# barlettacarmen/CrCNN

Hardware: AMD Instinct MI355X
Metric: encrypted images/sec (higher is better)
Workload: dtype u64

## Files before the change

crcnn_amd/csrc/abi.hip:

```cpp
#include <cstdlib>
#include <cstring>
#include "kernels.h"
#include "chacha.h"
#include "work_arena.h"

#define CHECK_CTX(c) do { if (!(c) || (c)->device < 0) return CRC_ERR_INVALID_ARGUMENT; \
        int dev_ = -1; if (hipGetDevice(&dev_) != hipSuccess || dev_ != (c)->device) HIPCHK(hipSetDevice((c)->device)); } while (0)
#define RUN(x) do { int rc_ = (x); if (rc_) return rc_; } while (0)
static inline hipStream_t S(void *s) { return (hipStream_t)s; }
static inline bool form_ok(int f) { return f == CRC_COEFF || f == CRC_NTT; }
static inline bool nform_ok(int f) { return f == CRC_COEFF || f == CRC_NTT || f == CRC_NTTP; }
static inline bool lform_ok(int f) { return nform_ok(f) || f == CRC_NTTL; }
static inline bool limb_in(int f) { return f == CRC_NTTL || f == CRC_NTTLS; }
static inline u64 *work_base(void *d_work) { return WorkArena(d_work).take<u64>(0); }
static inline size_t work_bytes(size_t words) { WorkArena a; a.take<u64>(words); return a.bytes(); }

extern "C" int crc_plain_to_ntt(crc_ctx *c, const uint64_t *d_plain, size_t count, uint64_t *d_out, void *stream)
{
    CHECK_CTX(c); if (!d_plain || !d_out) return CRC_ERR_INVALID_ARGUMENT;
    return k_plain_ntt(c, d_plain, count, 1, true, d_out, S(stream));
}
extern "C" int crc_plain_expand(crc_ctx *c, const uint64_t *d_compact, size_t count, uint64_t *d_plain, void *stream)
{
    CHECK_CTX(c); if (!d_compact || !d_plain) return CRC_ERR_INVALID_ARGUMENT;
// ... 324 lines not shown
    if (!d_w || !d_bias_ntt || !d_w_out || !d_bias_out || nf < 1 || zd < 1 || xf < 1 || yf < 1 || cxs < 1 || cys < 1 || pxf < 1 ||
        pyf < 1) return CRC_ERR_INVALID_ARGUMENT;
    return k_fold_pool(c, d_w, d_bias_ntt, d_div_ntt, d_w_out, d_bias_out, nf, zd, xf, yf, cxs, cys, pxf, pyf, S(stream));
}
extern "C" int crc_conv2d_hoist_pool(crc_ctx *c, const uint64_t *d_w, const uint64_t *d_bias_ntt, const uint64_t *d_div_ntt, int nf, int zd, int xf, int yf,
                                     int pxf, int pyf, uint64_t *d_w_out, uint64_t *d_bias_out, void *stream)
{
    CHECK_CTX(c);
    if (!d_w || !d_bias_ntt || !d_w_out || !d_bias_out || nf < 1 || zd < 1 || xf < 1 || yf < 1 || pxf < 1 || pyf < 1) return CRC_ERR_INVALID_ARGUMENT;
    return k_fold_pool(c, d_w, d_bias_ntt, d_div_ntt, d_w_out, d_bias_out, nf, zd, xf, yf, 1, 1, pxf, pyf, S(stream), true);
}

extern "C" int crc_pool(crc_ctx *c, const uint64_t *d_x, int B, int zd, int xd, int yd, int xs, int ys, int xf, int yf,
                        const uint64_t *d_div, int form, uint64_t *d_y, void *stream)
{
    CHECK_CTX(c);
    if (!d_x || !d_y || B < 0 || zd < 1 || !nform_ok(form) || !conv_shape_ok(xd, yd, xs, ys, xf, yf)) return CRC_ERR_INVALID_ARGUMENT;
    if (B == 0) return CRC_OK;
    hipStream_t st = S(stream);
    const int xo = (xd - xf) / xs + 1, yo = (yd - yf) / ys + 1;
    if (form == CRC_NTTP) return k_pool(c, d_x, d_y, B, zd, xd, yd, xs, ys, xf, yf, d_div, st, 1);
    if (form == CRC_NTT || !d_div) return k_pool(c, d_x, d_y, B, zd, xd, yd, xs, ys, xf, yf, form == CRC_NTT ? d_div : nullptr, st);
    RUN(k_pool(c, d_x, d_y, B, zd, xd, yd, xs, ys, xf, yf, nullptr, st));
    const size_t cnt = (size_t)B * zd * xo * yo;
    RUN(k_ntt_ct(c, false, d_y, d_y, cnt, 2, false, st, nullptr, 0, 0));
    RUN(k_rowwise(c, d_y, d_div, cnt, 2, 2, 1, cnt, 0, st));
    return k_ntt_ct(c, true, d_y, d_y, cnt, 2, false, st, nullptr, 0, 0);
}

extern "C" int crc_pad(crc_ctx *c, const uint64_t *d_x, int B, int zd, int xd, int yd, int px0, int px1, int py0, int py1, int form, uint64_t *d_y,
                       void *stream)
{
    CHECK_CTX(c);
    if (!d_x || !d_y || B < 0 || zd < 1 || xd < 1 || yd < 1 || px0 < 0 || px1 < 0 || py0 < 0 || py1 < 0 || !form_ok(form)) return CRC_ERR_INVALID_ARGUMENT;
    if (((uintptr_t)d_x | (uintptr_t)d_y) & 15) return CRC_ERR_INVALID_ARGUMENT;
    const long long xo = (long long)xd + px0 + px1, yo = (long long)yd + py0 + py1;
    if (xo > 0x7fffffffLL || yo > 0x7fffffffLL) return CRC_ERR_INVALID_ARGUMENT;
    const size_t ctb = crc_ct_words(c, 2) * 8;
    const size_t in_bytes = (size_t)B * zd * xd * yd * ctb, out_bytes = (size_t)B * zd * (size_t)xo * (size_t)yo * ctb;
    const uintptr_t x0 = (uintptr_t)d_x, y0 = (uintptr_t)d_y;
    if (x0 < y0 + out_bytes && y0 < x0 + in_bytes) return CRC_ERR_INVALID_ARGUMENT;
    if (B == 0) return CRC_OK;
    return k_pad(c, d_x, d_y, B, zd, xd, yd, px0, px1, py0, py1, S(stream));
}

extern "C" int crc_batchnorm(crc_ctx *c, uint64_t *d_x, int B, int zd, int xd, int yd, const uint64_t *d_mean, const uint64_t *d_invstd,
                             int form, void *stream)
{
    CHECK_CTX(c);
    if (!d_x || !d_mean || !d_invstd || B < 0 || zd < 1 || xd < 1 || yd < 1 || !form_ok(form)) return CRC_ERR_INVALID_ARGUMENT;
    if (B == 0) return CRC_OK;
    hipStream_t st = S(stream);
    const size_t hw = (size_t)xd * yd, cnt = (size_t)B * zd * hw;
    if (form == CRC_NTT) return k_bn_ntt(c, d_x, B, zd, (int)hw, d_mean, d_invstd, st);
    RUN(k_rowwise(c, d_x, d_mean, cnt, 2, 1, -1, hw, (size_t)zd, st));
    RUN(k_ntt_ct(c, false, d_x, d_x, cnt, 2, false, st, nullptr, 0, 0));
    RUN(k_rowwise(c, d_x, d_invstd, cnt, 2, 2, 1, hw, (size_t)zd, st));
    return k_ntt_ct(c, true, d_x, d_x, cnt, 2, false, st, nullptr, 0, 0);
}

extern "C" int crc_plan_mac(const crc_ctx *c, int zd, int xd, int yd, int xs, int ys, int xf, int yf, int nf, int B, int matrix_cores, int *w_form)
{
    if (!c || !w_form || zd < 1 || nf < 1 || !conv_shape_ok(xd, yd, xs, ys, xf, yf)) return CRC_ERR_INVALID_ARGUMENT;
    bool packable = true;
    for (int i = 0; i < c->k; i++) if (c->tabs[i].m.bits > 55) packable = false;
    *w_form = packable ? CRC_NTTP : CRC_NTT;
    if (!matrix_cores || !packable) return CRC_OK;
    if (zd == 1) { if (k_limb_conv1_shape(c, zd, xd, yd, xs, ys, xf, yf, nf)) *w_form = CRC_NTTL1; return CRC_OK; }
    const int min_steps = c->tune.mfma_min_steps > 0 ? c->tune.mfma_min_steps : 8;
    const long long P = (long long)((xd - xf) / xs + 1) * ((yd - yf) / ys + 1);
    const long long rows = (long long)B * 2 * P, min_rows = nf >= 24 ? 32 : 64;
    const bool few_filters_ok = nf >= 24 || (long long)c->n * c->k <= 32768;
    if (zd >= 16 && few_filters_ok && (long long)((zd + 31) / 32) * xf * yf >= min_steps && crc_limb_supported(c, zd, xf, yf) && (B <= 0 ||
        rows >= min_rows)) *w_form = CRC_NTTL;
    return CRC_OK;
}
extern "C" size_t crc_scalar_weights_bytes(const crc_ctx *c, int nf, int zd, int xf, int yf)
{
    return c && nf >= 1 && zd >= 1 && xf >= 1 && yf >= 1 ? k_scalar_weights_bytes(c, nf, zd, xf, yf) : 0;
}
extern "C" int crc_scalar_supported(const crc_ctx *c, int B, int zd, int xd, int yd, int xs, int ys, int xf, int yf, int nf)
{
    if (!c || B < 1 || zd < 1 || nf < 1 || !conv_shape_ok(xd, yd, xs, ys, xf, yf)) return 0;
    return k_scalar_supported(c, B, zd, xd, yd, xs, ys, xf, yf, nf) ? 1 : 0;
}
extern "C" int crc_scalar_pack_weights(crc_ctx *c, const uint64_t *d_w, int w_stride, int nf, int zd, int xf, int yf, void *d_ws, int *constant, void *stream)
{
    if (constant) *constant = 1;
    CHECK_CTX(c);
    if (!d_w || !d_ws || !constant || nf < 1 || zd < 1 || xf < 1 || yf < 1 || (w_stride != 1 && w_stride != c->n)) return CRC_ERR_INVALID_ARGUMENT;
    if (c->k > 8 || !k_limb_supported(c, k_limb_steps(zd, xf, yf) * 32)) return CRC_ERR_UNSUPPORTED;
    return k_scalar_pack_weights(c, d_w, (size_t)w_stride, (signed char *)d_ws, nf, zd, xf, yf, constant, S(stream));
}
extern "C" int crc_plan_mac_scalar(const crc_ctx *c, int zd, int xd, int yd, int xs, int ys, int xf, int yf, int nf, int B, int *w_form)
{
    RUN(crc_plan_mac(c, zd, xd, yd, xs, ys, xf, yf, nf, B, 1, w_form));
    if (c->tune.scalar_mac && zd >= 2 && k_scalar_supported(c, B < 1 ? 1 : B, zd, xd, yd, xs, ys, xf, yf, nf)) *w_form = CRC_NTTLS;
    return CRC_OK;
}
extern "C" int crc_plan_fold_pool(const crc_ctx *c, int zd, int xd, int yd, int xs, int ys, int xf, int yf, int nf, int pxs, int pys, int pxf, int pyf,
    int *fold)
{
    if (!c || !fold || zd < 1 || nf < 1 || !conv_shape_ok(xd, yd, xs, ys, xf, yf) || pxs < 1 || pys < 1 || pxf < 1 || pyf < 1) return CRC_ERR_INVALID_ARGUMENT;
    *fold = 0;
    const int xo = (xd - xf) / xs + 1, yo = (yd - yf) / ys + 1;
    const int xf2 = (pxf - 1) * xs + xf, yf2 = (pyf - 1) * ys + yf, xs2 = xs * pxs, ys2 = ys * pys;
    if (xf2 > xd || yf2 > yd || pxf > xo || pyf > yo) return CRC_OK;
    const int xo2 = (xd - xf2) / xs2 + 1, yo2 = (yd - yf2) / ys2 + 1;
    if (xo2 != (xo - pxf) / pxs + 1 || yo2 != (yo - pyf) / pys + 1) return CRC_OK;
    const long long fpad = (nf + 7) / 8 * 8, T1 = (long long)zd * xf * yf, T2 = (long long)zd * xf2 * yf2;
    const long long cost_sep = fpad * xo * yo * (T1 + 24) + (long long)nf * xo2 * yo2 * 10 * (pxf * pyf + 1);
    const long long cost_fused = fpad * xo2 * yo2 * (T2 + 24);
    *fold = cost_fused < cost_sep ? 1 : 0;
    return CRC_OK;
}

static long long plan_mac_cost(const crc_ctx *c, int zd, int xd, int yd, int xs, int ys, int xf, int yf, int nf, int B, int matrix_cores)
{
    int wf = CRC_NTT;
    if (crc_plan_mac(c, zd, xd, yd, xs, ys, xf, yf, nf, B, matrix_cores, &wf) != CRC_OK) return -1;
    const long long P = (long long)((xd - xf) / xs + 1) * ((yd - yf) / ys + 1);
    if (wf == CRC_NTTL1) return 32 * ((2 * P + 15) / 16 * 8) * ((k_limb_conv1_form(c, xf, yf, nf) == 2 ? 40 : 64) + 24) * 8 / 5;
    if (wf == CRC_NTTL) return (long long)(nf + 31) / 32 * 32 * P * ((long long)k_limb_steps(zd, xf, yf) * 32 + 24);
    return (long long)(nf + 7) / 8 * 8 * P * ((long long)zd * xf * yf + 24);
}
extern "C" int crc_plan_hoist_pool(const crc_ctx *c, int uzd, int uxd, int uyd, int uxs, int uys, int uxf, int uyf, int unf, int zd, int xd, int yd, int xs,
                                   int ys, int xf, int yf, int nf, int pxs, int pys, int pxf, int pyf, int B, int matrix_cores, int *hoist)
{
    if (!c || !hoist || zd < 1 || nf < 1 || !conv_shape_ok(xd, yd, xs, ys, xf, yf) || pxs < 1 || pys < 1 || pxf < 1 || pyf < 1) return CRC_ERR_INVALID_ARGUMENT;
    *hoist = 0;
    if (!c->tune.hoist_pool || xs != 1 || ys != 1 || pxs * pys == 1) return CRC_OK;
    int fold = 0;
    { const int rc = crc_plan_fold_pool(c, zd, xd, yd, xs, ys, xf, yf, nf, pxs, pys, pxf, pyf, &fold); if (rc != CRC_OK) return rc; }
    if (!fold) return CRC_OK;
    if (uzd < 1 || unf != zd || !conv_shape_ok(uxd, uyd, uxs, uys, uxf, uyf) || (uxd - uxf) / uxs + 1 != xd || (uyd - uyf) / uys + 1 != yd) return CRC_OK;
    const int uxf2 = (pxf - 1) * uxs + uxf, uyf2 = (pyf - 1) * uys + uyf, sxd = xd - pxf + 1, syd = yd - pyf + 1;
    if (uxf2 > uxd || uyf2 > uyd || !conv_shape_ok(uxd, uyd, uxs, uys, uxf2, uyf2)) return CRC_OK;
    if ((uxd - uxf2) / uxs + 1 != sxd || (uyd - uyf2) / uys + 1 != syd) return CRC_OK;
    const int xo = xd - xf + 1, yo = yd - yf + 1;
    if (!conv_shape_ok(sxd, syd, pxs, pys, xf, yf) || (sxd - xf) / pxs + 1 != (xo - pxf) / pxs + 1 || (syd - yf) / pys + 1 != (yo - pyf) / pys + 1) return CRC_OK;
    int uf = CRC_NTT, uf2 = CRC_NTT;
    if (crc_plan_mac(c, uzd, uxd, uyd, uxs, uys, uxf, uyf, unf, B, matrix_cores, &uf) != CRC_OK) return CRC_OK;
    if (crc_plan_mac(c, uzd, uxd, uyd, uxs, uys, uxf2, uyf2, unf, B, matrix_cores, &uf2) != CRC_OK) return CRC_OK;
    if ((uf == CRC_NTTL1 || uf == CRC_NTTL) && uf2 != uf) return CRC_OK;
    const int xf2 = xf + pxf - 1, yf2 = yf + pyf - 1;
    const long long folded = plan_mac_cost(c, uzd, uxd, uyd, uxs, uys, uxf, uyf, unf, B, matrix_cores) +
                             plan_mac_cost(c, zd, xd, yd, pxs, pys, xf2, yf2, nf, B, matrix_cores);
    const long long hoisted = plan_mac_cost(c, uzd, uxd, uyd, uxs, uys, uxf2, uyf2, unf, B, matrix_cores) +
                              plan_mac_cost(c, zd, sxd, syd, pxs, pys, xf, yf, nf, B, matrix_cores);
    *hoist = hoisted < folded ? 1 : 0;
    return CRC_OK;
}

#define PLAN_BOX_READ 21
extern "C" int crc_plan_conv1_box(const crc_ctx *c, int zd, int xd, int yd, int xs, int ys, int xf, int yf, int nf, int bxf, int byf, int B, int matrix_cores,
                                  int *box)
{
    if (!c || !box || zd < 1 || nf < 1 || bxf < 1 || byf < 1 || !conv_shape_ok(xd, yd, xs, ys, xf, yf)) return CRC_ERR_INVALID_ARGUMENT;
    *box = 0;
    if (!c->tune.conv1_box || !matrix_cores || bxf * byf == 1) return CRC_OK;
    if (!crc_limb_conv1_box_supported(c, zd, xd, yd, xs, ys, xf, yf, nf, bxf, byf)) return CRC_OK;
    const int xf2 = (bxf - 1) * xs + xf, yf2 = (byf - 1) * ys + yf, xdi = xd - (bxf - 1) * xs, ydi = yd - (byf - 1) * ys;
    if (!conv_shape_ok(xd, yd, xs, ys, xf2, yf2)) return CRC_OK;
    int wf = CRC_NTT;
    if (crc_plan_mac(c, zd, xdi, ydi, xs, ys, xf, yf, nf, B, matrix_cores, &wf) != CRC_OK || wf != CRC_NTTL1) return CRC_OK;
    const long long enlarged = plan_mac_cost(c, zd, xd, yd, xs, ys, xf2, yf2, nf, B, matrix_cores);
    const long long boxed = plan_mac_cost(c, zd, xdi, ydi, xs, ys, xf, yf, nf, B, matrix_cores) +
                            (long long)xdi * ydi * 2 * (bxf * byf - 1) * PLAN_BOX_READ;
    *box = enlarged >= 0 && boxed < enlarged ? 1 : 0;
    return CRC_OK;
}

static size_t square_chunk(const crc_ctx *c)
{
    if (c->tune.sq_chunk > 0) return (size_t)c->tune.sq_chunk;
    const size_t nk = (size_t)c->n * c->k;
    return nk <= 32768 ? 1024 : nk <= 65536 ? 512 : nk <= 131072 ? 256 : 128;
}

struct ActWork { u64 *xh, *s, *kp, *y3, *rest; size_t step; };
enum { ACT_XH = 1, ACT_S = 2, ACT_MULTIPLY = 4 };
static ActWork act_layout(const crc_ctx *c, size_t planes, size_t pin, size_t pout, int dbc, int regions, WorkArena &a)
{
    ActWork L{};
    L.step = square_chunk(c) / pin ? square_chunk(c) / pin : 1;
    const size_t pp = planes < L.step ? planes : L.step, cin = pp * pin, cout = pp * pout;
    const size_t pr = regions & ACT_MULTIPLY ? k_multiply_work_words(c, cin) : k_square_work_words(c, cin), rl = k_relin_work_words(c, cout, dbc);
    if (regions & ACT_XH) L.xh = a.take<u64>(cin * crc_ct_words(c, 2));
    if (regions & ACT_S) L.s = a.take<u64>(cin * crc_ct_words(c, 2));
    L.kp = a.take<u64>(k_relin_keys_words(c, dbc));
    L.y3 = a.take<u64>(cin * crc_ct_words(c, 3));
    L.rest = a.take<u64>(pr > rl ? pr : rl);
    return L;
}
static size_t act_bytes(const crc_ctx *c, size_t planes, size_t pin, size_t pout, int dbc, int regions)
{
    WorkArena a;
    act_layout(c, planes, pin, pout, dbc, regions, a);
    return a.bytes();
}
static inline size_t pass_len(size_t count, size_t o, size_t step) { return count - o < step ? count - o : step; }
static int ntt_copy(crc_ctx *c, const u64 *x, size_t ch, u64 *xh, void *stream)
{
    HIPCHK(hipMemcpyAsync(xh, x, 8 * ch * crc_ct_words(c, 2), hipMemcpyDeviceToDevice, S(stream)));
    return crc_ntt_fwd(c, xh, ch, 2, stream);
}
extern "C" size_t crc_square_relin_work_bytes(const crc_ctx *c, size_t count, int dbc) { return c && dbc_ok(dbc) ? act_bytes(c, count, 1, 1, dbc, 0) : 0; }
extern "C" size_t crc_encrypt_dev_work_bytes(const crc_ctx *c, size_t count) { return c ? work_bytes(k_encrypt_work_words(c, count)) : 0; }
extern "C" int crc_encrypt_dev_key(crc_ctx *c, const uint64_t *d_pk, const uint64_t *d_plain, size_t count, const uint8_t *key, uint64_t stream_base,
                                   uint64_t *d_ct, void *d_work, void *stream)
{
    return crc_encrypt_dev_key_forms(c, d_pk, d_plain, count, key, stream_base, CRC_COEFF, d_ct, d_work, stream);
}
extern "C" int crc_encrypt_dev(crc_ctx *c, const uint64_t *d_pk, const uint64_t *d_plain, size_t count, uint64_t seed, uint64_t *d_ct, void *d_work,
    void *stream)
{
    return crc_encrypt_dev_forms(c, d_pk, d_plain, count, seed, CRC_COEFF, d_ct, d_work, stream);
}
extern "C" int crc_encrypt_dev_key_forms(crc_ctx *c, const uint64_t *d_pk, const uint64_t *d_plain, size_t count, const uint8_t *key, uint64_t stream_base,
                                         int out_form, uint64_t *d_ct, void *d_work, void *stream)
{
    CHECK_CTX(c); if (!d_pk || !d_plain || !d_ct || !d_work || !key || (out_form != CRC_COEFF && out_form != CRC_NTT)) return CRC_ERR_INVALID_ARGUMENT;
    return k_encrypt(c, d_pk, d_plain, count, chacha_load_key(key), stream_base, d_ct, work_base(d_work), S(stream), out_form == CRC_NTT);
}
extern "C" int crc_encrypt_dev_forms(crc_ctx *c, const uint64_t *d_pk, const uint64_t *d_plain, size_t count, uint64_t seed, int out_form, uint64_t *d_ct,
                                     void *d_work, void *stream)
{
    CHECK_CTX(c); if (!d_pk || !d_plain || !d_ct || !d_work || (out_form != CRC_COEFF && out_form != CRC_NTT)) return CRC_ERR_INVALID_ARGUMENT;
    return k_encrypt(c, d_pk, d_plain, count, chacha_seed_key(seed), 0, d_ct, work_base(d_work), S(stream), out_form == CRC_NTT);
}
extern "C" void crc_encrypt_dev_noise_thresholds(uint64_t *h_out19) { if (h_out19) k_encrypt_cdt(h_out19); }

static bool ct_form_ok(int f) { return f == CRC_COEFF || f == CRC_NTT; }
extern "C" size_t crc_decrypt_dev_work_bytes(const crc_ctx *c, size_t count, int size, int in_form)
{
    return c && ct_form_ok(in_form) ? work_bytes(k_decrypt_work_words(c, count, size, in_form == CRC_NTT)) : 0;
}
extern "C" int crc_decrypt_dev(crc_ctx *c, const uint64_t *d_sk, const uint64_t *d_ct, size_t count, int size, int in_form, uint64_t *d_plain, void *d_work,
                               void *stream)
{
    CHECK_CTX(c); if (!d_sk || !d_ct || !d_plain || !d_work || !ct_form_ok(in_form)) return CRC_ERR_INVALID_ARGUMENT;
    return k_decrypt(c, d_sk, d_ct, count, size, in_form == CRC_NTT, d_plain, work_base(d_work), S(stream));
}
extern "C" size_t crc_noise_budget_dev_work_bytes(const crc_ctx *c, size_t count, int size, int in_form)
{
    return c && ct_form_ok(in_form) && (size == 2 || size == 3) ? work_bytes(k_decrypt_work_words(c, count, size, in_form == CRC_NTT)) : 0;
}
extern "C" int crc_noise_budget_dev(crc_ctx *c, const uint64_t *d_sk, const uint64_t *d_ct, size_t count, int size, int in_form, int32_t *d_bits, int32_t *d_min,
                                    void *d_work, void *stream)
{
    if (!d_sk || !d_ct || !d_bits || !d_work || !ct_form_ok(in_form) || size < 2 || size > 3) return CRC_ERR_INVALID_ARGUMENT;
    CHECK_CTX(c);
    return k_noise_budget(c, d_sk, d_ct, count, size, in_form == CRC_NTT, d_bits, d_min, work_base(d_work), S(stream));
}
extern "C" int crc_budget_bits_host(const crc_ctx *c, const uint64_t *h_v, size_t count, int32_t *h_bits)
{
    if (!c || !h_v || !h_bits) return CRC_ERR_INVALID_ARGUMENT;
    return k_budget_bits_host(c, h_v, count, h_bits);
}
static int slots_args_ok(const crc_ctx *c, const void *values, const void *plain, int slots, size_t item_stride, size_t slot_stride)
{
    if (!crc_slots_supported(c)) return CRC_ERR_PARAMETERS;
    if (!values || !plain || slots < 1 || slots > c->n || !item_stride || !slot_stride) return CRC_ERR_INVALID_ARGUMENT;
    return CRC_OK;
}
extern "C" int crc_slots_compose(crc_ctx *c, const int64_t *h_values, size_t count, int slots, size_t item_stride, size_t slot_stride, uint64_t *h_plain)
{
    if (!c) return CRC_ERR_INVALID_ARGUMENT;
    RUN(slots_args_ok(c, h_values, h_plain, slots, item_stride, slot_stride));
    return k_slots_compose_host(c, (const long long *)h_values, count, slots, item_stride, slot_stride, h_plain);
}
extern "C" int crc_slots_decompose(crc_ctx *c, const uint64_t *h_plain, size_t count, int slots, int64_t *h_values, size_t item_stride, size_t slot_stride)
{
    if (!c) return CRC_ERR_INVALID_ARGUMENT;
    RUN(slots_args_ok(c, h_values, h_plain, slots, item_stride, slot_stride));
    return k_slots_decompose_host(c, h_plain, count, slots, (long long *)h_values, item_stride, slot_stride);
}
extern "C" int crc_slots_compose_dev(crc_ctx *c, const int64_t *d_values, size_t count, int slots, size_t item_stride, size_t slot_stride, uint64_t *d_plain,
                                     void *stream)
{
    CHECK_CTX(c);
    RUN(slots_args_ok(c, d_values, d_plain, slots, item_stride, slot_stride));
    if (((uintptr_t)d_plain & 15) || ((uintptr_t)d_values & 7)) return CRC_ERR_INVALID_ARGUMENT;
    return k_slots_compose(c, (const long long *)d_values, count, slots, item_stride, slot_stride, d_plain, S(stream));
}
extern "C" int crc_slots_decompose_dev(crc_ctx *c, const uint64_t *d_plain, size_t count, int slots, int64_t *d_values, size_t item_stride, size_t slot_stride,
                                       void *stream)
{
    CHECK_CTX(c);
    RUN(slots_args_ok(c, d_values, d_plain, slots, item_stride, slot_stride));
    if (((uintptr_t)d_plain & 15) || ((uintptr_t)d_values & 7)) return CRC_ERR_INVALID_ARGUMENT;
    return k_slots_decompose(c, d_plain, count, slots, (long long *)d_values, item_stride, slot_stride, S(stream));
}
static int slots_rescale_args_ok(const crc_ctx *c, const void *in, const void *out, uint64_t divisor)
{
    if (!crc_slots_supported(c)) return CRC_ERR_PARAMETERS;
    if (!in || !out || divisor < 1 || divisor > ((uint64_t)1 << 62)) return CRC_ERR_INVALID_ARGUMENT;
    return CRC_OK;
}
extern "C" int crc_slots_rescale(crc_ctx *c, const uint64_t *h_plain_in, size_t count, uint64_t divisor, uint64_t *h_plain_out)
{
    if (!c) return CRC_ERR_INVALID_ARGUMENT;
    RUN(slots_rescale_args_ok(c, h_plain_in, h_plain_out, divisor));
    return k_slots_rescale_host(c, h_plain_in, count, divisor, h_plain_out);
}
extern "C" int crc_slots_rescale_dev(crc_ctx *c, const uint64_t *d_plain_in, size_t count, uint64_t divisor, uint64_t *d_plain_out, void *stream)
{
// ... 401 lines not shown
```

crcnn_amd/csrc/kernels_mfma1.hip:

```cpp
#include "kernels.h"
#include "limbred.h"
#include <cstdlib>

typedef int v4i __attribute__((ext_vector_type(4)));
typedef signed char i8;
#define NPL 7
#define MAXK 8

struct Conv1Args {
    const i8 *xr; const i8 *wl; u64 *ys; i8 *xl_out; const ModParams *mods; const u64 *bias;
    int n, k, B, Bout, b0, xd, yo, xs, ystr, P, F, mtiles;
    unsigned img_stride, plane_bytes, poly_bytes;
    unsigned out_img_bytes;
    int out_zdc;
    int narrow;
    int acc0[MAXK][13];
    u32 qbits[MAXK], qfold[MAXK];
    unsigned px_rs;
    int px_taps, px_yf, px_pair;
    int acc7[MAXK][7];
};

__device__ __forceinline__ void limb_digits1(u64 r, u64 q, int (&d)[NPL])
{
    long long v = r > (q >> 1) ? (long long)r - (long long)q : (long long)r;
#pragma unroll
    for (int l = 0; l < NPL; l++) { d[l] = (int)(signed char)(v & 0xff); v = (v - d[l]) >> 8; }
}

__device__ __forceinline__ void conv1_store4(const Conv1Args &a, i8 *stage, const long long (&cv)[4], int mm, int f0, int chan_bytes, u64 q, int slot, int b)
{
    if (mm >= 2 * a.P) return;
    if (a.xl_out) {
        if (f0 >= chan_bytes) return;
        u32 lo[4], hi[4];
#pragma unroll
        for (int reg = 0; reg < 4; reg++) { const u64 dg = f0 + reg < a.F ? centred_digit_bytes(cv[reg]) : 0; lo[reg] = (u32)dg;
            hi[reg] = (u32)(dg >> 32); }
        const u32 t0 = __builtin_amdgcn_perm(lo[1], lo[0], 0x05010400u), t1 = __builtin_amdgcn_perm(lo[1], lo[0], 0x07030602u);
        const u32 u0 = __builtin_amdgcn_perm(lo[3], lo[2], 0x05010400u), u1 = __builtin_amdgcn_perm(lo[3], lo[2], 0x07030602u);
        const u32 t2 = __builtin_amdgcn_perm(hi[1], hi[0], 0x05010400u), t3 = __builtin_amdgcn_perm(hi[1], hi[0], 0x07030602u);
        const u32 u2 = __builtin_amdgcn_perm(hi[3], hi[2], 0x05010400u), u3 = __builtin_amdgcn_perm(hi[3], hi[2], 0x07030602u);
        u32 pl[NPL];
        pl[0] = __builtin_amdgcn_perm(u0, t0, 0x05040100u); pl[1] = __builtin_amdgcn_perm(u0, t0, 0x07060302u);
        pl[2] = __builtin_amdgcn_perm(u1, t1, 0x05040100u); pl[3] = __builtin_amdgcn_perm(u1, t1, 0x07060302u);
        pl[4] = __builtin_amdgcn_perm(u2, t2, 0x05040100u); pl[5] = __builtin_amdgcn_perm(u2, t2, 0x07060302u);
        pl[6] = __builtin_amdgcn_perm(u3, t3, 0x05040100u);
        i8 *sp; unsigned pstride;
        if (a.out_zdc) { sp = stage + ((mm & 1) * a.P + (mm >> 1)) * a.out_zdc + f0; pstride = 2 * a.P * a.out_zdc; }
        else { sp = stage + mm * (NPL * 32) + f0; pstride = 32; }
#pragma unroll
        for (int l = 0; l < NPL; l++) *reinterpret_cast<u32 *>(sp + l * pstride) = pl[l];
    } else {
#pragma unroll
        for (int reg = 0; reg < 4; reg++)
            if (f0 + reg < a.F) a.ys[(((size_t)slot * a.B + b) * a.F + f0 + reg) * (2 * a.P) + mm] = (u64)(cv[reg] + ((cv[reg] >> 63) & (long long)q));
    }
}
__device__ __forceinline__ void conv1_copy_out(const Conv1Args &a, const i8 *stage, int slot, int b)
{
    i8 *dst = a.xl_out + ((size_t)slot * a.Bout + a.b0 + b) * a.out_img_bytes;
    if (a.out_zdc) {
        for (unsigned o = threadIdx.x; o < a.out_img_bytes / 16; o += blockDim.x)
            *reinterpret_cast<uint4 *>(dst + (size_t)o * 16) = *reinterpret_cast<const uint4 *>(stage + (size_t)o * 16);
    } else {
        const unsigned per_plane = a.out_img_bytes / (NPL * 16);
        for (unsigned o = threadIdx.x; o < NPL * per_plane; o += blockDim.x) {
            const unsigned l = o / per_plane, rem = o - l * per_plane;
            *reinterpret_cast<uint4 *>(dst + (size_t)o * 16) = *reinterpret_cast<const uint4 *>(stage + (rem >> 1) * (NPL * 32) + l * 32 +
                (rem & 1) * 16);
        }
    }
}

__global__ void __launch_bounds__(768) mfma_conv1_kernel(Conv1Args a)
{
    extern __shared__ __attribute__((aligned(16))) i8 lds[];
    const int lane = threadIdx.x & 63, wave = __builtin_amdgcn_readfirstlane(threadIdx.x >> 6), nwaves = blockDim.x >> 6;
    const int slot = blockIdx.x, i = slot / a.n, s = slot % a.n;
    const u64 q = a.mods[i].q;
    const u32 qbits = a.qbits[i], qfold = a.qfold[i];
    const int g = lane >> 4, r16 = lane & 15;
    const bool narrow = a.narrow != 0;
    const int nt = narrow ? (wave >> 2) & 1 : wave & 1;
    const int tile0 = !narrow ? wave >> 1 : nt ? wave - 4 : (wave < 4 ? wave : wave - 4), tile_step = !narrow ? nwaves >> 1 : nt ? 4 : nwaves - 4;
    const bool nar = narrow && nt;
    v4i wv[NPL];
    {
        const i8 *ws = a.wl + (size_t)slot * (NPL * 32 * 64) + (nt * 16 + r16) * 64 + g * 16;
        if (!nar) {
#pragma unroll
            for (int l = 0; l < NPL; l++) wv[l] = *reinterpret_cast<const v4i *>(ws + l * (32 * 64));
        } else {
            const i8 *wp = a.wl + (size_t)slot * (NPL * 32 * 64) + (16 + (r16 >> 2)) * 64 + g * 16;
#pragma unroll
            for (int grp = 0; grp < 2; grp++) {
                const int pl = 4 * grp + (r16 & 3);
                wv[grp] = pl < NPL ? *reinterpret_cast<const v4i *>(wp + pl * (32 * 64)) : v4i{0, 0, 0, 0};
            }
#pragma unroll
            for (int l = 2; l < NPL; l++) wv[l] = v4i{0, 0, 0, 0};
        }
    }
    u32 PB[7];
#pragma unroll
    for (int j = 0; j < 6; j++) PB[j] = (u32)a.acc0[i][2 * j] + ((u32)a.acc0[i][2 * j + 1] << 8);
    PB[6] = (u32)a.acc0[i][12];
    const u32 rcp_yo = (65536u + (u32)a.yo - 1) / (u32)a.yo;
    const int f0 = nt * 16 + 4 * g;
    long long bvc[4];
#pragma unroll
    for (int reg = 0; reg < 4; reg++) {
        const int f = f0 + reg;
        const u64 bv = (a.bias && f < a.F && !(lane & 1)) ? a.bias[((size_t)f * a.k + i) * a.n + s] : 0;
        bvc[reg] = bv > (q >> 1) ? (long long)(bv - q) : (long long)bv;
    }
    long long bvn = 0;
    if (nar) {
        const int f = 16 + g;
        const u64 bv = (a.bias && f < a.F && !(lane & 1)) ? a.bias[((size_t)f * a.k + i) * a.n + s] : 0;
        bvn = bv > (q >> 1) ? (long long)(bv - q) : (long long)bv;
    }
    i8 *stage = lds + 2 * (size_t)a.img_stride;
    const i8 *ximg = a.xr + (size_t)slot * a.B * a.img_stride;
    const int pieces = a.img_stride / 1024;
    auto issue_img = [&](int b) {
        i8 *dst = lds + (b & 1) * (size_t)a.img_stride;
        const i8 *src = ximg + (size_t)b * a.img_stride + lane * 16;
        for (int pc = wave; pc < pieces; pc += nwaves)
            __builtin_amdgcn_global_load_lds((const __attribute__((address_space(1))) void *)(src + pc * 1024),
                (__attribute__((address_space(3))) void *)(dst + pc * 1024), 16, 0, 0);
    };
    if (a.xl_out && a.out_zdc && threadIdx.x < 16) { const unsigned e = a.out_img_bytes - 16 + threadIdx.x;
        if (e >= (unsigned)(NPL * 2 * a.P * a.out_zdc)) stage[e] = 0; }
    issue_img(0);
    const int chan_bytes = a.out_zdc ? a.out_zdc : 32;
    for (int b = 0; b < a.B; b++) {
        __builtin_amdgcn_s_waitcnt(0 | (7 << 4) | (15 << 8));
        __syncthreads();
        if (b + 1 < a.B) issue_img(b + 1);
        const i8 *img = lds + (b & 1) * (size_t)a.img_stride;
        for (int mt = tile0; mt < a.mtiles; mt += tile_step) {
            v4i acc[13];
#pragma unroll
            for (int d = 0; d < 13; d++) acc[d] = v4i{0, 0, 0, 0};
            const int mm = mt * 16 + r16, mrow = min(mm, 2 * a.P - 1), p = mrow >> 1, c = mrow & 1, ox = (int)(((u32)p * rcp_yo) >> 16), oy = p - ox * a.yo;
            const int r0 = min(ox * a.xs + 2 * g, a.xd - 1), r1 = min(ox * a.xs + 2 * g + 1, a.xd - 1);
            const int off = oy * a.ystr, sh = off & 3;
            const i8 *p0 = img + c * a.poly_bytes + (off & ~3) + r0 * 32, *p1 = img + c * a.poly_bytes + (off & ~3) + r1 * 32;
            auto window = [&](int l) {
                const u32 *q0 = reinterpret_cast<const u32 *>(p0 + l * a.plane_bytes), *q1 = reinterpret_cast<const u32 *>(p1 + l * a.plane_bytes);
                const u32 a0 = q0[0], a1 = q0[1], a2 = q0[2], b0 = q1[0], b1 = q1[1], b2 = q1[2];
                return v4i{(int)__builtin_amdgcn_alignbyte(a1, a0, sh), (int)__builtin_amdgcn_alignbyte(a2, a1, sh), (int)__builtin_amdgcn_alignbyte(b1, b0,
                    sh),
// ... 110 lines not shown
        if (e >= (unsigned)(NPL * 2 * a.P * a.out_zdc)) stage[e] = 0; }
    issue_img(0);
    const int chan_bytes = a.out_zdc ? a.out_zdc : 32;
    for (int b = 0; b < a.B; b++) {
        __builtin_amdgcn_s_waitcnt(0 | (7 << 4) | (15 << 8));
        __syncthreads();
        if (b + 1 < a.B) issue_img(b + 1);
        const i8 *img = lds + (b & 1) * (size_t)a.img_stride;
        for (int mt = tile0; mt < a.mtiles; mt += tile_step) {
            const int mm = mt * 16 + r16, mrow = min(mm, 2 * a.P - 1), p = mrow >> 1, c = mrow & 1, ox = (int)(((u32)p * rcp_yo) >> 16), oy = p - ox * a.yo;
            const i8 *win = img + c * a.poly_bytes + (u32)(ox * a.xs) * a.px_rs + (u32)(oy * a.ystr) * 8;
            v4i bv[NJ];
            if (a.px_pair) {
#pragma unroll
                for (int j = 0; j < NJ; j++) bv[j] = *reinterpret_cast<const v4i *>(win + (toff[j] & 0xffffu));
            } else {
#pragma unroll
                for (int j = 0; j < NJ; j++) {
                    const uint2 t0 = *reinterpret_cast<const uint2 *>(win + (toff[j] & 0xffffu)), t1 = *reinterpret_cast<const uint2 *>(win + (toff[j] >> 16));
                    bv[j] = v4i{(int)t0.x, (int)t0.y, (int)t1.x, (int)t1.y};
                }
            }
            v4i acc[NPL];
#pragma unroll
            for (int m = 0; m < NPL; m++) acc[m] = __builtin_amdgcn_mfma_i32_16x16x64_i8(wv[m][0], bv[0], v4i{0, 0, 0, 0}, 0, 0, 0);
#pragma unroll
            for (int j = 1; j < NJ; j++)
#pragma unroll
                for (int m = 0; m < NPL; m++) acc[m] = __builtin_amdgcn_mfma_i32_16x16x64_i8(wv[m][j], bv[j], acc[m], 0, 0, 0);
            long long cv[4];
#pragma unroll
            for (int reg = 0; reg < 4; reg++) {
                int E[NPL];
#pragma unroll
                for (int m = 0; m < NPL; m++) E[m] = acc[m][reg];
                cv[reg] = diag7_fold_centred(E, q, qbits, qfold, bvc[reg], PB);
            }
            conv1_store4(a, stage, cv, mm, f0, chan_bytes, q, slot, b);
        }
        if (a.xl_out) {
            __syncthreads();
            conv1_copy_out(a, stage, slot, b);
        }
    }
}

#define RG 4
#define RSL 32
__global__ void __launch_bounds__(256) limb_pack_rows1_kernel(const u64 *x, i8 *xr, const ModParams *mods, int n, int k, int B, int xd, int yd, int packed,
                                                              unsigned img_stride, unsigned plane_bytes, unsigned poly_bytes)
{
    __shared__ __attribute__((aligned(16))) i8 st[RSL * NPL * RG * 32];
    const int sblocks = n / RSL;
    const int sb = blockIdx.x % (sblocks * k), i = sb / sblocks, s0 = (sb % sblocks) * RSL;
    const int rgs = (xd + RG - 1) / RG;
    size_t r = blockIdx.x / (sblocks * k);
    const int rg = (int)(r % rgs); r /= rgs; const int c = (int)(r % 2); const int b = (int)(r / 2);
    const u64 q = mods[i].q;
    const int lane = threadIdx.x & (RSL - 1), qrow = (threadIdx.x >> 5) & (RG - 1), h = threadIdx.x >> 7, row = rg * RG + qrow;
    {
        u32 pl[NPL][4];
#pragma unroll
        for (int l = 0; l < NPL; l++)
#pragma unroll
            for (int wv = 0; wv < 4; wv++) pl[l][wv] = 0;
        if (row < xd) {
            const u64 *src = x + ((((size_t)b * xd * yd + (size_t)row * yd + h * 16) * 2 + c) * k + i) * (size_t)n + s0 + lane;
#pragma unroll
            for (int colx = 0; colx < 16; colx++)
                if (h * 16 + colx < yd) {
                    u64 v = src[(size_t)colx * 2 * k * n];
                    if (packed) v = (v & 0xffffffffULL) | ((v >> 32) << 28);
                    const u64 dg = balanced_digit_bytes(v, q);
#pragma unroll
                    for (int l = 0; l < NPL; l++) pl[l][colx >> 2] |= (u32)((dg >> (8 * l)) & 0xff) << (8 * (colx & 3));
                }
        }
        i8 *sp = st + (size_t)lane * (NPL * RG * 32) + qrow * 32 + h * 16;
#pragma unroll
        for (int l = 0; l < NPL; l++) *reinterpret_cast<uint4 *>(sp + l * (RG * 32)) = make_uint4(pl[l][0], pl[l][1], pl[l][2], pl[l][3]);
    }
    __syncthreads();
    const int pieces_per_run = RG * 2, rows_here = min(RG, xd - rg * RG);
    for (int o = threadIdx.x; o < RSL * NPL * pieces_per_run; o += 256) {
        const int run = o / pieces_per_run, part = o - run * pieces_per_run, sl = run / NPL, l = run - sl * NPL;
        if ((part >> 1) >= rows_here) continue;
        i8 *dst = xr + (((size_t)i * n + s0 + sl) * B + b) * img_stride + (size_t)l * plane_bytes + (size_t)c * poly_bytes + (size_t)(rg * RG) * 32 + part * 16;
        *reinterpret_cast<uint4 *>(dst) = *reinterpret_cast<const uint4 *>(st + (size_t)run * (RG * 32) + part * 16);
    }
}
template <bool BOX>
__global__ void __launch_bounds__(256) limb_pack_rows1_kernel_px(const u64 *x, i8 *xr, const ModParams *mods, int n, int k, int B, int xd, int yd, int packed,
                                                                 unsigned img_stride, unsigned poly_bytes, unsigned rs, int xdo, int ydo, int bxf, int byf, int xs,
                                                                 int ys)
{
    extern __shared__ __attribute__((aligned(16))) i8 stp[];
    const unsigned sstride = RG * rs + 16;
    const int sblocks = n / RSL;
    const int sb = blockIdx.x % (sblocks * k), i = sb / sblocks, s0 = (sb % sblocks) * RSL;
    const int rgs = (xdo + RG - 1) / RG;
    size_t r = blockIdx.x / (sblocks * k);
    const int rg = (int)(r % rgs); r /= rgs; const int c = (int)(r % 2); const int b = (int)(r / 2);
    const u64 q = mods[i].q;
    const int lane = threadIdx.x & (RSL - 1), qrow = (threadIdx.x >> 5) & (RG - 1), h = threadIdx.x >> 7, row = rg * RG + qrow;
    if (row < xdo) {
        const size_t cs = (size_t)2 * k * n;
        const u64 *src = x + ((((size_t)b * xd * yd + (size_t)row * yd + h * 16) * 2 + c) * k + i) * (size_t)n + s0 + lane;
        u64 *sp = reinterpret_cast<u64 *>(stp + (size_t)lane * sstride + qrow * rs) + h * 16;
        if constexpr (!BOX) {
#pragma unroll
            for (int colx = 0; colx < 16; colx++) {
                const int col = h * 16 + colx;
                if ((unsigned)col * 8 >= rs) continue;
                u64 dg = 0;
                if (col < yd) {
                    u64 v = src[(size_t)colx * cs];
                    if (packed) v = (v & 0xffffffffULL) | ((v >> 32) << 28);
                    dg = balanced_digit_bytes(v, q);
                }
                sp[colx] = dg;
            }
        } else {
            u64 sum[16];
#pragma unroll
            for (int colx = 0; colx < 16; colx++) sum[colx] = 0;
            for (int a = 0; a < bxf; a++)
                for (int bb = 0; bb < byf; bb++) {
                    const u64 *tp = src + ((size_t)a * xs * yd + (size_t)bb * ys) * cs;
#pragma unroll
                    for (int colx = 0; colx < 16; colx++)
                        if (h * 16 + colx < ydo) {
                            u64 v = tp[(size_t)colx * cs];
                            if (packed) v = (v & 0xffffffffULL) | ((v >> 32) << 28);
                            sum[colx] += v;
                        }
                }
#pragma unroll
            for (int colx = 0; colx < 16; colx++) {
                const int col = h * 16 + colx;
                if ((unsigned)col * 8 >= rs) continue;
                sp[colx] = col < ydo ? balanced_digit_bytes(sum_reduce16(sum[colx], q), q) : 0;
            }
        }
    }
    __syncthreads();
    const int per_run = RG * rs / 16, valid = min(RG, xdo - rg * RG) * (int)rs / 16;
    for (int o = threadIdx.x; o < RSL * per_run; o += 256) {
        const int sl = o / per_run, part = o - sl * per_run;
        if (part >= valid) continue;
        i8 *dst = xr + (((size_t)i * n + s0 + sl) * B + b) * img_stride + (size_t)c * poly_bytes + (size_t)(rg * RG) * rs + part * 16;
        *reinterpret_cast<uint4 *>(dst) = *reinterpret_cast<const uint4 *>(stp + (size_t)sl * sstride + part * 16);
    }
}
__global__ void __launch_bounds__(64) limb_pack_w1_kernel(const u64 *w, i8 *wl, const ModParams *mods, int n, int k, int F, int xf, int yf)
{
    const int sblocks = n / 64;
    const int sb = blockIdx.x % (sblocks * k), i = sb / sblocks, s = (sb % sblocks) * 64 + threadIdx.x;
    size_t r = blockIdx.x / (sblocks * k);
    const int ky = (int)(r % yf); r /= yf; const int kx = (int)(r % xf); const int f = (int)(r / xf);
    const ModParams m = mods[i];
    int d[NPL]; limb_digits1(w[((((size_t)f * xf + kx) * yf + ky) * k + i) * (size_t)n + s], m.q, d);
    i8 *dst = wl + ((size_t)i * n + s) * (NPL * 32 * 64) + f * 64 + kx * 8 + ky;
#pragma unroll
    for (int l = 0; l < NPL; l++) dst[(size_t)l * (32 * 64)] = (i8)d[l];
}

__global__ void __launch_bounds__(64) limb_pack_w1_kernel_px(const u64 *w, i8 *wl, const ModParams *mods, int n, int k, int F, int xf, int yf)
{
    const int sblocks = n / 64;
    const int sb = blockIdx.x % (sblocks * k), i = sb / sblocks, s = (sb % sblocks) * 64 + threadIdx.x;
    size_t r = blockIdx.x / (sblocks * k);
    const int ky = (int)(r % yf); r /= yf; const int kx = (int)(r % xf); const int f = (int)(r / xf);
    const ModParams m = mods[i];
    u64 v = w[((((size_t)f * xf + kx) * yf + ky) * k + i) * (size_t)n + s];
    const int tap = kx * yf + ky, G = tap >> 1;
    i8 *dst = wl + ((size_t)i * n + s) * (NPL * NJ * 32 * 64) + ((G >> 2) * 32 + f) * 64 + (G & 3) * 16 + (tap & 1) * 8;
    for (int l = 0; l < NPL; l++) {
        int d[NPL]; limb_digits1(v, m.q, d);
#pragma unroll
        for (int dm = 0; dm < NPL; dm++) dst[(size_t)dm * (NJ * 32 * 64) + l] = (i8)d[dm];
        v = mulmod(v, 256, m);
    }
}

static inline unsigned conv1_poly_bytes(int xd) { return ((unsigned)xd + 1) * 32; }
static inline unsigned conv1_img_stride(int xd) { const unsigned b = NPL * 2 * conv1_poly_bytes(xd); return (b + 1023) / 1024 * 1024; }
static inline unsigned conv1_px_rs(int yd) { return ((unsigned)yd * 8 + 15) / 16 * 16; }
static inline unsigned conv1_px_poly_bytes(int xd, int yd) { const unsigned b = (unsigned)xd * conv1_px_rs(yd); return b + (128 + 256 - b % 256) % 256; }
static inline unsigned conv1_px_img_stride(int xd, int yd) { return (2 * conv1_px_poly_bytes(xd, yd) + 1023) / 1024 * 1024; }
static bool conv1_fits(unsigned img_stride, int xd, int yd, int xs, int ys_, int xf, int yf)
{
    const int xo = (xd - xf) / xs + 1, yo = (yd - yf) / ys_ + 1;
    return 2 * (size_t)img_stride + (size_t)NPL * xo * yo * 2 * 32 <= 160 * 1024;
}
int k_limb_conv1_form(const crc_ctx *c, int xf, int yf, int nf)
{
    bool px = xf * yf <= 8 * NJ;
    for (int i = 0; i < c->k && px; i++) px = conv1_fold7_ok(c->tabs[i].m.q, c->tabs[i].m.bits, fold_constant(c->tabs[i].m.q, c->tabs[i].m.bits));
    const int forced = c->tune.conv1_form;
    if (forced == 1 || !px) return 1;
    if (forced == 2) return 2;
    return nf > 16 && nf <= 20 ? 1 : 2;
}
bool k_limb_conv1_shape(const crc_ctx *c, int zd, int xd, int yd, int xs, int ys_, int xf, int yf, int nf)
{
    if (zd != 1 || xf > 8 || yf > 8 || nf > 32 || yd > 32 || c->n < 64 || c->k > MAXK) return false;
    for (int i = 0; i < c->k; i++) if (!conv1_fold_ok(c->tabs[i].m.q, c->tabs[i].m.bits, fold_constant(c->tabs[i].m.q, c->tabs[i].m.bits))) return false;
    const int xo = (xd - xf) / xs + 1, yo = (yd - yf) / ys_ + 1;
    if (xo * yo > 1024) return false;
    return conv1_fits(k_limb_conv1_form(c, xf, yf, nf) == 2 ? conv1_px_img_stride(xd, yd) : conv1_img_stride(xd), xd, yd, xs, ys_, xf, yf);
}
bool k_limb_conv1_box_shape(const crc_ctx *c, int zd, int xd, int yd, int xs, int ys_, int xf, int yf, int nf, int bxf, int byf)
{
    if (bxf < 1 || byf < 1 || bxf * byf > 9) return false;
    const int xdo = xd - (bxf - 1) * xs, ydo = yd - (byf - 1) * ys_;
    if (xdo < xf || ydo < yf || !k_limb_conv1_shape(c, zd, xdo, ydo, xs, ys_, xf, yf, nf)) return false;
    return bxf * byf == 1 || k_limb_conv1_form(c, xf, yf, nf) == 2;
}
static size_t conv1_form_weights_bytes(const crc_ctx *c, int form) { return (size_t)c->n * c->k * NPL * 32 * 64 * (form == 2 ? NJ : 1); }
size_t k_limb_conv1_weights_bytes(const crc_ctx *c) { return conv1_form_weights_bytes(c, 2); }
size_t k_limb_conv1_weights_bytes_for(const crc_ctx *c, int nf, int xf, int yf) { return conv1_form_weights_bytes(c, k_limb_conv1_form(c, xf, yf, nf)); }
size_t k_limb_conv1_image_bytes(const crc_ctx *c, int B, int xd, int yd, int xf, int yf, int nf)
{
    return (size_t)c->n * c->k * B * (k_limb_conv1_form(c, xf, yf, nf) == 2 ? conv1_px_img_stride(xd, yd) : conv1_img_stride(xd));
}

static void conv1_tables(const crc_ctx *c, Conv1Args &a)
{
    for (int i = 0; i < c->k; i++) { conv1_bias_table(c->tabs[i].m.q, a.acc0[i]); conv1_bias7_table(c->tabs[i].m.q, a.acc7[i]); a.qbits[i] = c->tabs[i].m.bits;
        a.qfold[i] = fold_constant(c->tabs[i].m.q, c->tabs[i].m.bits); }
}

int k_limb_conv1_pack_weights(crc_ctx *c, const u64 *w, i8 *wl, int nf, int xf, int yf, hipStream_t st)
{
    const int form = k_limb_conv1_form(c, xf, yf, nf);
    HIPCHK(hipMemsetAsync(wl, 0, conv1_form_weights_bytes(c, form), st));
    const size_t blocks = (size_t)(c->n / 64) * c->k * nf * xf * yf;
    if (form == 2) hipLaunchKernelGGL(limb_pack_w1_kernel_px, dim3((unsigned)blocks), dim3(64), 0, st, w, wl, c->d_mods, c->n, c->k, nf, xf, yf);
    else hipLaunchKernelGGL(limb_pack_w1_kernel, dim3((unsigned)blocks), dim3(64), 0, st, w, wl, c->d_mods, c->n, c->k, nf, xf, yf);
    HIPCHK(hipGetLastError());
    return CRC_OK;
}
int k_limb_conv1(crc_ctx *c, const u64 *x, bool packed, i8 *xr, const i8 *wl, u64 *ys, i8 *xl_out, int Bout, int b0, const u64 *bias_ntt, int B, int xd_in,
    int yd_in, int xs, int ys_,
                 int xf, int yf, int nf, hipStream_t st, int bxf, int byf)
{
    if (B == 0) return CRC_OK;
    if (!k_limb_conv1_box_shape(c, 1, xd_in, yd_in, xs, ys_, xf, yf, nf, bxf, byf)) return CRC_ERR_UNSUPPORTED;
    const int xd = xd_in - (bxf - 1) * xs, yd = yd_in - (byf - 1) * ys_;
    const int xo = (xd - xf) / xs + 1, yo = (yd - yf) / ys_ + 1;
    const int form = k_limb_conv1_form(c, xf, yf, nf);
    Conv1Args a{};
    a.xr = xr; a.wl = wl; a.ys = ys; a.xl_out = xl_out; a.mods = c->d_mods; a.bias = bias_ntt;
    a.n = c->n; a.k = c->k; a.B = B; a.Bout = Bout; a.b0 = b0; a.xd = xd; a.yo = yo; a.xs = xs; a.ystr = ys_; a.P = xo * yo; a.F = nf;
        a.mtiles = (2 * a.P + 15) / 16;
    a.out_zdc = a.P > 1 ? k_limb_flat_zdc(nf) : 0;
    a.out_img_bytes = a.out_zdc ? (unsigned)((NPL * 2 * a.P * a.out_zdc + 15) / 16 * 16) : (unsigned)(NPL * a.P * 2 * 32);
    conv1_tables(c, a);
    const size_t pack_blocks = (size_t)(c->n / RSL) * c->k * B * 2 * ((xd + RG - 1) / RG);
    if (pack_blocks > 0x7fffffffULL) return CRC_ERR_INVALID_ARGUMENT;
    if (form == 2) {
        a.px_rs = conv1_px_rs(yd); a.poly_bytes = conv1_px_poly_bytes(xd, yd); a.img_stride = conv1_px_img_stride(xd, yd);
        a.px_taps = xf * yf; a.px_yf = yf;
        a.px_pair = yf % 2 == 0 && ys_ % 2 == 0 ? 1 : 0;
        if (bxf * byf > 1)
            hipLaunchKernelGGL(limb_pack_rows1_kernel_px<true>, dim3((unsigned)pack_blocks), dim3(256), RSL * (RG * a.px_rs + 16), st, x, xr, c->d_mods, c->n, c->k,
                B, xd_in, yd_in, packed ? 1 : 0, a.img_stride, a.poly_bytes, a.px_rs, xd, yd, bxf, byf, xs, ys_);
        else
            hipLaunchKernelGGL(limb_pack_rows1_kernel_px<false>, dim3((unsigned)pack_blocks), dim3(256), RSL * (RG * a.px_rs + 16), st, x, xr, c->d_mods, c->n, c->k,
                B, xd_in, yd_in, packed ? 1 : 0, a.img_stride, a.poly_bytes, a.px_rs, xd, yd, 1, 1, xs, ys_);
        HIPCHK(hipGetLastError());
        const size_t lds = 2 * (size_t)a.img_stride + (xl_out ? a.out_img_bytes : 0);
        { const int rc = crc_ctx_ensure_lds(c, (const void *)mfma_conv1_kernel_px, lds); if (rc) return rc; }
        hipLaunchKernelGGL(mfma_conv1_kernel_px, dim3((unsigned)(c->n * c->k)), dim3(64 * 8), lds, st, a);
        HIPCHK(hipGetLastError());
        return CRC_OK;
    }
    a.poly_bytes = conv1_poly_bytes(xd); a.plane_bytes = 2 * a.poly_bytes; a.img_stride = conv1_img_stride(xd);
    a.narrow = c->tune.conv1_narrow != 0 && nf > 16 && nf <= 20 ? 1 : 0;
    {
        hipLaunchKernelGGL(limb_pack_rows1_kernel, dim3((unsigned)pack_blocks), dim3(256), 0, st, x, xr, c->d_mods, c->n, c->k, B, xd, yd, packed ? 1 : 0,
            a.img_stride, a.plane_bytes,
                           a.poly_bytes);
        HIPCHK(hipGetLastError());
    }
    auto busiest = [&](int nw) {
        int load[4] = {0, 0, 0, 0}, worst = 0;
        for (int w = 0; w < nw; w++) load[w & 3] += (a.mtiles - (w >> 1) + nw / 2 - 1) / (nw / 2);
        for (int sd = 0; sd < 4; sd++) worst = load[sd] > worst ? load[sd] : worst;
        return worst;
    };
    const int forced = c->tune.conv1_waves;
    const int nwaves = forced ? forced : a.narrow ? 12 : busiest(12) <= busiest(8) ? 12 : 8;
    const size_t lds = 2 * (size_t)a.img_stride + (xl_out ? a.out_img_bytes : 0);
    { const int rc = crc_ctx_ensure_lds(c, (const void *)mfma_conv1_kernel, lds); if (rc) return rc; }
    hipLaunchKernelGGL(mfma_conv1_kernel, dim3((unsigned)(c->n * c->k)), dim3(64 * nwaves), lds, st, a);
    HIPCHK(hipGetLastError());
    return CRC_OK;
}
```

Measured before the change: 792.0.

## Stage box-filter input rows in an LDS ring buffer for conv1 packing

Adds a pack kernel for the box-pooled conv1 path that loads each input row once into a shared-memory ring buffer and computes the box sum from LDS. The previous kernel re-read overlapping global input for every box tap. Each workgroup now walks all row groups of an image serially, which cuts the grid size and may reduce parallelism. The planner's box read-cost constant is also lowered, so the box path gets chosen more often.

```diff
diff --git a/crcnn_amd/csrc/abi.hip b/crcnn_amd/csrc/abi.hip
--- a/crcnn_amd/csrc/abi.hip
+++ b/crcnn_amd/csrc/abi.hip
@@ -500,7 +500,7 @@
     return CRC_OK;
 }
 
-#define PLAN_BOX_READ 21
+#define PLAN_BOX_READ 12
 extern "C" int crc_plan_conv1_box(const crc_ctx *c, int zd, int xd, int yd, int xs, int ys, int xf, int yf, int nf, int bxf, int byf, int B, int matrix_cores,
                                   int *box)
 {
diff --git a/crcnn_amd/csrc/boxstage.h b/crcnn_amd/csrc/boxstage.h
--- /dev/null
+++ b/crcnn_amd/csrc/boxstage.h
@@ -0,0 +1,40 @@
+#pragma once
+#include "modarith.h"
+
+#define BOX_RG 4
+#define BOX_RSL 32
+#define BOX_LDS_MAX (160 * 1024)
+
+CRC_HD int box_halo(int bxf, int xs) { return (bxf - 1) * xs; }
+CRC_HD int box_ring_rows(int bxf, int xs) { return BOX_RG + box_halo(bxf, xs); }
+CRC_HD u32 box_ring_px(int yd, int bxf, int xs) { return (u32)box_ring_rows(bxf, xs) * (u32)yd; }
+CRC_HD size_t box_ring_bytes(int yd, int bxf, int xs) { return (size_t)box_ring_px(yd, bxf, xs) * BOX_RSL * 8; }
+CRC_HD size_t box_digit_bytes(unsigned rs) { return (size_t)BOX_RSL * (BOX_RG * rs + 16); }
+CRC_HD size_t box_lds_bytes(int yd, int bxf, int xs, unsigned rs) { return box_ring_bytes(yd, bxf, xs) + box_digit_bytes(rs); }
+CRC_HD bool box_staged(int yd, int bxf, int xs, unsigned rs) { return box_lds_bytes(yd, bxf, xs, rs) <= BOX_LDS_MAX; }
+
+CRC_HD int box_row_groups(int xdo) { return (xdo + BOX_RG - 1) / BOX_RG; }
+CRC_HD int box_rows_here(int g, int xdo) { return xdo - g * BOX_RG < BOX_RG ? xdo - g * BOX_RG : BOX_RG; }
+CRC_HD int box_groups_per_wg(int xdo, int wpi) { return (box_row_groups(xdo) + wpi - 1) / wpi; }
+CRC_HD int box_walk_first(int w, int xdo, int wpi) { return w * box_groups_per_wg(xdo, wpi); }
+CRC_HD int box_walk_end(int w, int xdo, int wpi)
+{
+    const int e = (w + 1) * box_groups_per_wg(xdo, wpi), rgs = box_row_groups(xdo);
+    return e < rgs ? e : rgs;
+}
+CRC_HD int box_load_end(int g, int xd, int yd, int bxf, int xs)
+{
+    const int r = g * BOX_RG + box_ring_rows(bxf, xs);
+    return (r < xd ? r : xd) * yd;
+}
+CRC_HD int box_load_first(int g, bool walk_start, int xd, int yd, int bxf, int xs)
+{
+    const int f = (g * BOX_RG + (walk_start ? 0 : box_halo(bxf, xs))) * yd, e = box_load_end(g, xd, yd, bxf, xs);
+    return f < e ? f : e;
+}
+CRC_HD u32 box_cell(u32 px, u32 ring_px, int slot) { return (px % ring_px) * BOX_RSL + (u32)slot; }
+CRC_HD u32 box_ring_pos(u32 px, u32 ring_px) { return px % ring_px; }
+CRC_HD u32 box_ring_step(u32 pos, u32 step, u32 ring_px) { return pos + step >= ring_px ? pos + step - ring_px : pos + step; }
+CRC_HD u32 box_pos_cell(u32 pos, int slot) { return pos * BOX_RSL + (u32)slot; }
+CRC_HD int box_col(int h, int colx) { return h * 16 + colx; }
+CRC_HD u32 box_term_px(int row, int col, int a, int bb, int xs, int ys, int yd) { return (u32)((row + a * xs) * yd + col + bb * ys); }
diff --git a/crcnn_amd/csrc/kernels_mfma1.hip b/crcnn_amd/csrc/kernels_mfma1.hip
--- a/crcnn_amd/csrc/kernels_mfma1.hip
+++ b/crcnn_amd/csrc/kernels_mfma1.hip
@@ -1,5 +1,6 @@
 #include "kernels.h"
 #include "limbred.h"
+#include "boxstage.h"
 #include <cstdlib>
 
 typedef int v4i __attribute__((ext_vector_type(4)));
@@ -416,6 +417,74 @@
         *reinterpret_cast<uint4 *>(dst) = *reinterpret_cast<const uint4 *>(stp + (size_t)sl * sstride + part * 16);
     }
 }
+#define BOX_LD 16
+static_assert(BOX_RG == RG && BOX_RSL == RSL, "boxstage.h describes this pack's workgroup");
+__global__ void __launch_bounds__(256) limb_pack_box_kernel_px(const u64 *x, i8 *xr, const ModParams *mods, int n, int k, int B, int xd, int yd, int packed,
+                                                               unsigned img_stride, unsigned poly_bytes, unsigned rs, int xdo, int ydo, int bxf, int byf, int xs,
+                                                               int ys)
+{
+    extern __shared__ __attribute__((aligned(16))) i8 stp[];
+    u64 *ring = reinterpret_cast<u64 *>(stp);
+    i8 *dig = stp + box_ring_bytes(yd, bxf, xs);
+    const unsigned sstride = RG * rs + 16;
+    const int sblocks = n / RSL;
+    const int sb = blockIdx.x % (sblocks * k), i = sb / sblocks, s0 = (sb % sblocks) * RSL;
+    const int wpi = (int)(gridDim.x / (unsigned)(sblocks * k * 2 * B));
+    size_t r = blockIdx.x / (sblocks * k);
+    const int w = (int)(r % wpi); r /= wpi; const int c = (int)(r % 2); const int b = (int)(r / 2);
+    const u64 q = mods[i].q;
+    const int lane = threadIdx.x & (RSL - 1), seg = threadIdx.x >> 5, qrow = seg & (RG - 1), h = threadIdx.x >> 7;
+    const u32 ring_px = box_ring_px(yd, bxf, xs);
+    const size_t cs = (size_t)2 * k * n;
+    const u64 *src = x + (((size_t)b * xd * yd * 2 + c) * k + i) * (size_t)n + s0 + lane;
+    const int g0 = box_walk_first(w, xdo, wpi), g1 = box_walk_end(w, xdo, wpi);
+    for (int g = g0; g < g1; g++) {
+        const int p1 = box_load_end(g, xd, yd, bxf, xs);
+        for (int pb = box_load_first(g, g == g0, xd, yd, bxf, xs) + seg; pb < p1; pb += 8 * BOX_LD) {
+            u64 v[BOX_LD];
+#pragma unroll
+            for (int u = 0; u < BOX_LD; u++) v[u] = pb + 8 * u < p1 ? src[(size_t)(pb + 8 * u) * cs] : 0;
+#pragma unroll
+            for (int u = 0; u < BOX_LD; u++)
+                if (pb + 8 * u < p1) {
+                    u64 t = v[u];
+                    if (packed) t = (t & 0xffffffffULL) | ((t >> 32) << 28);
+                    ring[box_cell((u32)(pb + 8 * u), ring_px, lane)] = t;
+                }
+        }
+        __syncthreads();
+        const int row = g * RG + qrow;
+        if (row < xdo) {
+            u64 sum[16];
+#pragma unroll
+            for (int colx = 0; colx < 16; colx++) sum[colx] = 0;
+            for (int a = 0; a < bxf; a++)
+                for (int bb = 0; bb < byf; bb++) {
+                    u32 pos = box_ring_pos(box_term_px(row, box_col(h, 0), a, bb, xs, ys, yd), ring_px);
+#pragma unroll
+                    for (int colx = 0; colx < 16; colx++) {
+                        if (box_col(h, colx) < ydo) sum[colx] += ring[box_pos_cell(pos, lane)];
+                        pos = box_ring_step(pos, 1, ring_px);
+                    }
+                }
+            u64 *sp = reinterpret_cast<u64 *>(dig + (size_t)lane * sstride + qrow * rs) + h * 16;
+#pragma unroll
+            for (int colx = 0; colx < 16; colx++) {
+                const int col = box_col(h, colx);
+                if ((unsigned)col * 8 >= rs) continue;
+                sp[colx] = col < ydo ? balanced_digit_bytes(sum_reduce16(sum[colx], q), q) : 0;
+            }
+        }
+        __syncthreads();
+        const int per_run = RG * rs / 16, valid = box_rows_here(g, xdo) * (int)rs / 16;
+        for (int o = threadIdx.x; o < RSL * per_run; o += 256) {
+            const int sl = o / per_run, part = o - sl * per_run;
+            if (part >= valid) continue;
+            i8 *dst = xr + (((size_t)i * n + s0 + sl) * B + b) * img_stride + (size_t)c * poly_bytes + (size_t)(g * RG) * rs + part * 16;
+            *reinterpret_cast<uint4 *>(dst) = *reinterpret_cast<const uint4 *>(dig + (size_t)sl * sstride + part * 16);
+        }
+    }
+}
 __global__ void __launch_bounds__(64) limb_pack_w1_kernel(const u64 *w, i8 *wl, const ModParams *mods, int n, int k, int F, int xf, int yf)
 {
     const int sblocks = n / 64;
@@ -527,7 +596,13 @@
         a.px_rs = conv1_px_rs(yd); a.poly_bytes = conv1_px_poly_bytes(xd, yd); a.img_stride = conv1_px_img_stride(xd, yd);
         a.px_taps = xf * yf; a.px_yf = yf;
         a.px_pair = yf % 2 == 0 && ys_ % 2 == 0 ? 1 : 0;
-        if (bxf * byf > 1)
+        if (bxf * byf > 1 && box_staged(yd_in, bxf, xs, a.px_rs)) {
+            const size_t lds = box_lds_bytes(yd_in, bxf, xs, a.px_rs);
+            const int wpi = 1;
+            { const int rc = crc_ctx_ensure_lds(c, (const void *)limb_pack_box_kernel_px, lds); if (rc) return rc; }
+            hipLaunchKernelGGL(limb_pack_box_kernel_px, dim3((unsigned)((size_t)(c->n / RSL) * c->k * B * 2 * wpi)), dim3(256), lds, st, x, xr, c->d_mods, c->n,
+                c->k, B, xd_in, yd_in, packed ? 1 : 0, a.img_stride, a.poly_bytes, a.px_rs, xd, yd, bxf, byf, xs, ys_);
+        } else if (bxf * byf > 1)
             hipLaunchKernelGGL(limb_pack_rows1_kernel_px<true>, dim3((unsigned)pack_blocks), dim3(256), RSL * (RG * a.px_rs + 16), st, x, xr, c->d_mods, c->n, c->k,
                 B, xd_in, yd_in, packed ? 1 : 0, a.img_stride, a.poly_bytes, a.px_rs, xd, yd, bxf, byf, xs, ys_);
         else
```

Measured after the change: 807.3, median of 6. 1.02x the previous value.
